# google/dynibar

Measured on NVIDIA H100. Metric: rays/sec (64+64 samples x 8 src views), higher is better.
Workload: dtype bf16

## Files before the change

dynibar_b200/csrc/chains_wg.cu:

```cuda
#include "nets.cuh"
#include "wg_engine.cuh"

namespace dyn {

using namespace tc;
using namespace fe;
using namespace wg;

namespace {

constexpr float kLog2e = 1.4426950408889634f, kLn2 = 0.6931471805599453f;

template <int RING>
struct ChainBars {
  static constexpr int kTileFull = 2 * RING, kTileEmpty = 2 * RING + 1, kCount = 2 * RING + 2;
};

template <int kTile, int kExtra, int kConst, int RING = kWgRing>
struct ChainSmem {
  static constexpr int kTileOff = RING * kWgStage;
  static constexpr int kExtraOff = kTileOff + kTile;
  static constexpr int kConstOff = kExtraOff + kExtra;
  static constexpr int kBarOff = (kConstOff + kConst * 4 + 7) & ~7;
  static constexpr int kBytes = kBarOff + ChainBars<RING>::kCount * 8;
  static_assert(kBytes + kWgMaxChunks * 16 <= 227 * 1024, "shared memory of one CTA");
};

template <int RING = kWgRing>
__device__ __forceinline__ uint32_t chain_init(uint8_t* smem, int bar_off, FusedChunk* s_tab,
                                               const FusedChunk* chunks, int nchunks) {
  const uint32_t bar0 = smem_u32(smem + bar_off);
  stage_chunks(s_tab, chunks, nchunks);
  if (threadIdx.x == 0) {
    for (int i = 0; i < RING; ++i) {
      mbar_init(bar0 + 8u * i, 1);
      mbar_init(bar0 + 8u * (RING + i), 8);
    }
    mbar_init(bar0 + 8u * ChainBars<RING>::kTileFull, 1);
    mbar_init(bar0 + 8u * ChainBars<RING>::kTileEmpty, 8);
    mbar_fence_init();
  }
  return bar0;
}

template <int RING = kWgRing>
__device__ __forceinline__ void chain_producers(const FusedChunk* s_tab, int nchunks, const void* wimg,
                                                const void* src, uint32_t tile_bytes, int n_iter, uint8_t* smem,
                                                uint32_t bar0) {
  setmaxnreg_dec<kProducerRegs>();
  const int t = threadIdx.x & 127;
  if (t == 0) {
    producer_loop<RING, kWgStage>(s_tab, nchunks, wimg, n_iter, smem, bar0);
  } else if (t == 32) {
    const uint8_t* s = reinterpret_cast<const uint8_t*>(src);
    const uint32_t dst = smem_u32(smem + RING * kWgStage);
    uint32_t k = 0;
    for (int it = blockIdx.x; it < n_iter; it += gridDim.x, ++k) {
      if (k > 0) mbar_wait(bar0 + 8u * ChainBars<RING>::kTileEmpty, (k - 1) & 1);
      mbar_arrive_expect_tx(bar0 + 8u * ChainBars<RING>::kTileFull, tile_bytes);
      bulk_g2s(dst, s + (size_t)it * tile_bytes, tile_bytes, bar0 + 8u * ChainBars<RING>::kTileFull);
    }
  }
}
template <int RING = kWgRing>
__device__ __forceinline__ void tile_wait(uint32_t bar0, uint32_t k) {
  mbar_wait(bar0 + 8u * ChainBars<RING>::kTileFull, k & 1);
}
template <int RING = kWgRing>
__device__ __forceinline__ void tile_release(uint32_t bar0) {
  __syncwarp();
  if ((threadIdx.x & 31) == 0) mbar_arrive(bar0 + 8u * ChainBars<RING>::kTileEmpty);
}

__device__ __forceinline__ void bias_afrag(uint32_t* a, int c0, int q) {
  const uint32_t one = q == 0 ? 0x3F803F80u : 0u;
  a[0] = a[1] = c0 == 0 ? one : 0u;
  a[2] = a[3] = c0 == 0 ? 0u : one;
}
template <int NA>
__device__ __forceinline__ void elu_log2_all(float* acc) {
#pragma unroll
  for (int i = 0; i < NA; ++i) acc[i] = elu_log2(acc[i]);
}

__device__ __forceinline__ float2* f32_pair(const void* base, long long row, int c) {
  return reinterpret_cast<float2*>(const_cast<uint8_t*>(reinterpret_cast<const uint8_t*>(base)) +
                                   tile_f32_off(row, c >> 2) + (c & 3) * 4);
}

__device__ __forceinline__ void store_image128(const float* acc, void* img, long long row0, const int* fr, int q,
                                               long long P) {
  uint8_t* o = reinterpret_cast<uint8_t*>(img);
#pragma unroll
  for (int h = 0; h < 2; ++h) {
    const long long row = row0 + fr[h];
    const bool ok = row < P;
#pragma unroll
    for (int j = 0; j < 16; ++j)
      *reinterpret_cast<uint32_t*>(o + tile_image_off(row, j, 16) + 4 * q) =
          ok ? pack_bf16x2(acc[4 * j + 2 * h], acc[4 * j + 2 * h + 1]) : 0u;
  }
}

__device__ __forceinline__ float rows8_max(float v) {
  v = fmaxf(v, __shfl_xor_sync(0xffffffffu, v, 4));
  v = fmaxf(v, __shfl_xor_sync(0xffffffffu, v, 8));
  return fmaxf(v, __shfl_xor_sync(0xffffffffu, v, 16));
}

constexpr int kP1Tile = 34 * 2048;
using P1Smem = ChainSmem<kP1Tile, 0, 0>;

__global__ void __launch_bounds__(kWgThreads, 1) point1_wg_kernel(const __grid_constant__ Point1Args a) {
  extern __shared__ __align__(1024) uint8_t smem[];
  __shared__ __align__(16) FusedChunk s_tab[kWgMaxChunks];
  const uint32_t bar0 = chain_init(smem, P1Smem::kBarOff, s_tab, a.chunks, a.nchunks);
  __syncthreads();
  const int n_iter = (int)((a.P + 127) / 128);
  const int tid = threadIdx.x, lane = tid & 31;
  const int wg = __shfl_sync(0xffffffffu, tid >> 7, 0);
  if (wg == 2) {
    chain_producers(s_tab, a.nchunks, a.wimg, a.G, (uint32_t)kP1Tile, n_iter, smem, bar0);
    return;
  }
  setmaxnreg_inc<kConsumerRegs>();
  const int q = lane & 3, ww = (tid & 127) >> 5;
  const int fr[2] = {16 * ww + (lane >> 2), 16 * ww + (lane >> 2) + 8};
  Ring rg{smem, bar0, 0u, false, 0};
  const uint32_t tile = smem_u32(smem + P1Smem::kTileOff) + 1024u * wg;
  uint32_t k = 0;
  for (int it = blockIdx.x; it < n_iter; it += gridDim.x, ++k) {
    const long long row0 = (long long)it * 128 + 64 * wg;
    float acc[128];
    tile_wait(bar0, k);
    layer_ss<256, 17, 128>(acc, tile, rg);
    layer_finish<256>(acc, rg);
    tile_release(bar0);
    {
      uint32_t af[17][4];
      elu_log2_all<128>(acc);
#pragma unroll
      for (int s = 0; s < 16; ++s) acc_to_afrag(acc, s, af[s]);
      bias_afrag(af[16], 8, q);
      layer_rs<128, 17>(acc, af, rg);
    }
#pragma unroll
    for (int h = 0; h < 2; ++h) {
      const long long row = row0 + fr[h];
      const bool ok = row < a.P;
      const float* pe = a.posenc ? a.posenc + (ok ? row % a.S : 0) * 128 : nullptr;
#pragma unroll
      for (int j = 0; j < 16; ++j) {
        const int c = 8 * j + 2 * q;
        float v0 = elu_from_log2(acc[4 * j + 2 * h]), v1 = elu_from_log2(acc[4 * j + 2 * h + 1]);
        if (pe) {
          const float2 p = __ldg(reinterpret_cast<const float2*>(pe + c));
          v0 += p.x;
          v1 += p.y;
        }
        acc[4 * j + 2 * h] = v0;
        acc[4 * j + 2 * h + 1] = v1;
        if (ok) *f32_pair(a.g2, row, c) = make_float2(v0, v1);
      }
    }
    uint32_t ag[8][4];
    to_afrag<8>(acc, ag);
    layer_rs<128, 8>(acc, ag, rg);
    store_image128(acc, a.Q, row0, fr, q, a.P);
    layer_rs<128, 8>(acc, ag, rg);
    store_image128(acc, a.K, row0, fr, q, a.P);
    layer_rs<128, 8>(acc, ag, rg);
    store_image128(acc, a.V, row0, fr, q, a.P);
  }
}

constexpr int kP2Tile = 16 * 2048;
constexpr int kPePtsBytes = 6 * 1024, kPeDirBytes = 4 * 1024;
constexpr int C_LNW = 0, C_LNB = 128, C_WOG2 = 256, C_WRGB4 = 384, C_BOG2 = 576, C_BRGB4 = 577;
constexpr int kP2Const = 580;
using P2Smem = ChainSmem<kP2Tile, 2 * (kPePtsBytes + kPeDirBytes), kP2Const>;

__device__ __forceinline__ void point2_constants(const Point2Args& a, float* cst, bool dynamic) {
  const int tid = threadIdx.x;
  const float* p = a.params;
  for (int i = tid; i < 128; i += blockDim.x) {
    cst[C_LNW + i] = p[a.o_lnw + i];
    cst[C_LNB + i] = p[a.o_lnb + i];
    cst[C_WOG2 + i] = p[a.o_woutgeo2 + i] * kLn2;
  }
  if (dynamic) {
    for (int i = tid; i < 192; i += blockDim.x) cst[C_WRGB4 + i] = p[a.o_wrgb4 + i] * kLn2;
    if (tid < 3) cst[C_BRGB4 + tid] = p[a.o_brgb4 + tid];
  }
  if (tid == 0) cst[C_BOG2] = p[a.o_boutgeo2];
}

__device__ __forceinline__ void write_pe_tiles(const Point2Args& a, long long row0, uint8_t* pe_pts, uint8_t* pe_dir) {
  const int tw = (threadIdx.x & 127) >> 6, r = threadIdx.x & 63;
  const long long row = row0 + r;
  const bool valid = row < a.P;
  if (tw == 0) {
    float p3[3] = {0.f, 0.f, 0.f};
    if (valid) { p3[0] = a.pts[row * 3]; p3[1] = a.pts[row * 3 + 1]; p3[2] = a.pts[row * 3 + 2]; }
    float pe[48];
    pe_pow2<3, 5>(p3, pe);
    pe[33] = 1.f; pe[34] = 1.f;
#pragma unroll
    for (int i = 35; i < 48; ++i) pe[i] = 0.f;
    uint8_t* arow = pe_pts + (r >> 3) * 128 + (r & 7) * 16;
#pragma unroll
    for (int g = 0; g < 6; ++g) store8_64(arow, 8 * g, pe + 8 * g);
  } else {
    const long long ray = valid ? row / a.S : 0;
    float d3[3] = {a.ray_dir[ray * 3], a.ray_dir[ray * 3 + 1], a.ray_dir[ray * 3 + 2]};
    float pe2[32];
    pe_pow2<3, 4>(d3, pe2);
    pe2[27] = 1.f; pe2[28] = 1.f;
#pragma unroll
    for (int i = 29; i < 32; ++i) pe2[i] = 0.f;
    uint8_t* arow = pe_dir + (r >> 3) * 128 + (r & 7) * 16;
#pragma unroll
    for (int g = 0; g < 4; ++g) store8_64(arow, 8 * g, pe2 + 8 * g);
  }
  fence_proxy_async_smem();
}

template <bool DYNAMIC, class RG>
__device__ __forceinline__ void point2_heads(float* acc, const Point2Args& a, const float* cst, uint32_t pe_pts,
                                             uint32_t pe_dir, const long long* rows, const bool* ok, const float* nv,
                                             int wg, RG& rg) {
  const int q = threadIdx.x & 3;
// ... 740 lines not shown
```

dynibar_b200/csrc/view_wg.cu:

```cuda
#include "geometry.cuh"
#include "nets.cuh"
#include "wg_engine.cuh"

namespace dyn {

using namespace tc;
using namespace fe;
using namespace wg;

namespace {

constexpr int kPeBytes = 14 * 1024, kPoolBytes = 30 * 1024, kWgATile = kPeBytes + kPoolBytes;
constexpr int C_B1 = 0, C_B2 = 256, C_B3 = 304, C_B4 = 560, C_B5 = 688, C_B6 = 816, C_W6V = 944, C_B7 = 1072,
              C_W8 = 1200, C_MISC = 1328, C_DFEAT = 1332, C_CAMS = 1372, C_W1 = 1628, C_MK = 1756, C_TGT = 1884;
constexpr int kWgConst = C_TGT + 3 * kMaxTargets;
constexpr int kViewBars = 2 * kWgRing + 4;
constexpr int kWgSmem = kWgRing * kWgStage + 2 * kWgATile + kWgConst * 4 + 4  + kViewBars * 8;
static_assert(kWgSmem + kWgMaxChunks * 16 <= 227 * 1024, "shared memory of one CTA");
constexpr int kViewThreads = 4 * 128;
constexpr int kViewConsumerRegs = 208, kViewFrontRegs = 72, kViewProducerRegs = 24;

enum Phase {
  PH_FRONT, PH_BAR, PH_WEIGHTS, PH_F1, PH_F1_EPI, PH_F2, PH_F2_EPI, PH_F3, PH_F3_EPI, PH_F4, PH_F4_EPI, PH_F5,
  PH_F5_EPI, PH_F6, PH_F6_EPI, PH_F7, PH_F7_EPI, PH_POOL2, PH_HANDOFF,
  PH_T = 28, PH_W = 29, PH_ITERS = 30, PH_LIFE = 31
};
constexpr int kPhaseSlots = 32;
__shared__ long long s_phase[3][kPhaseSlots];
struct PhaseClock {
  const ViewFusedArgs& a;
  int wg;
  __device__ __forceinline__ bool on() const { return a.dbg != nullptr && blockIdx.x == 0 && (threadIdx.x & 127) == 0; }
  __device__ __forceinline__ long long* c() const { return s_phase[wg]; }
  __device__ __forceinline__ void start() {
    if (!on()) return;
    for (int i = 0; i < kPhaseSlots; ++i) c()[i] = 0;
    c()[PH_T] = c()[PH_LIFE] = clock64();
  }
  __device__ __forceinline__ void mark(int ph, long long waits) {
    if (!on()) return;
    long long* s = c();
    const long long now = clock64();
    s[ph] += now - s[PH_T] - (waits - s[PH_W]);
    s[PH_WEIGHTS] += waits - s[PH_W];
    s[PH_T] = now;
    s[PH_W] = waits;
  }
  __device__ __forceinline__ void iteration() {
    if (on()) ++c()[PH_ITERS];
  }
  __device__ __forceinline__ void finish() {
    if (!on()) return;
    c()[PH_LIFE] = clock64() - c()[PH_LIFE];
    for (int i = 0; i < kPhaseSlots; ++i) a.dbg[kPhaseSlots * wg + i] = c()[i];
  }
};

__device__ __forceinline__ void pe_comp(float x, float* o) {
  float s, c;
  __sincosf(x, &s, &c);
  o[0] = x;
#pragma unroll
  for (int k = 0; k < 5; ++k) {
    o[1 + k] = c;
    o[6 + k] = s;
    const float s2 = 2.f * s * c, c2 = 1.f - 2.f * s * s;
    s = s2; c = c2;
  }
}

template <int KS>
__device__ __forceinline__ void layer_ss256(float* acc, uint32_t a_tile, Ring& rg) {
  layer_issue<256, KS>(acc, rg, [&](float* d, int ks, uint64_t bd, uint32_t sc) {
    const uint64_t ad = smem_desc(a_tile + ks * 2048u, 1024u, 128u);
    Wgmma<128, 0, 0>::mma(d, ad, bd, sc);
    Wgmma<128, 0, 0>::mma(d + 64, ad, bd + (2048u >> 4), sc);
  });
}

template <int N, int KS>
__device__ __forceinline__ void layer_rs_issue(float* acc, const uint32_t (&af)[KS][4], Ring& rg) {
  layer_issue<N, KS>(acc, rg, [&](float* d, int ks, uint64_t bd, uint32_t sc) { WgmmaRS<N>::mma(d, af[ks], bd, sc); });
}

__device__ __forceinline__ void named_bar_arrive(int id, int nthreads) {
  asm volatile("bar.arrive %0, %1;" ::"r"(id), "r"(nthreads) : "memory");
}

__device__ __forceinline__ void store2_64(uint8_t* tile, int r, int col, float x, float y) {
  *reinterpret_cast<uint32_t*>(tile + (col >> 3) * 1024 + (r >> 3) * 128 + (r & 7) * 16 + (col & 7) * 2) =
      pack_bf16x2(x, y);
}

template <int VP, bool ST, bool MC>
__device__ __forceinline__ void front_end(const ViewFusedArgs& a, const float* cst, int t, long long row0,
                                          uint8_t* pe_tile, uint8_t* pool_tile, float* s_w1, float* s_mk) {
  const int tw = t >> 6, r = t & 63, v = r & (VP - 1);
  uint8_t* arow_pe = pe_tile + (r >> 3) * 128 + (r & 7) * 16;
  uint8_t* arow_pool = pool_tile + (r >> 3) * 128 + (r & 7) * 16;
  const float wh = a.w_img, hh = a.h_img;
  const bool want_rgb = (tw == 0) || (ST && a.mask_rgb);

  const long long pl = (row0 + r) / VP;
  const bool pt_ok = pl < a.P;
  const bool valid = pt_ok && v < a.V;
  const long long m = pl * a.V + v;
  float p3[3] = {0.f, 0.f, 0.f};
  if (pt_ok) { p3[0] = a.pts[pl * 3]; p3[1] = a.pts[pl * 3 + 1]; p3[2] = a.pts[pl * 3 + 2]; }
  float q3[3] = {p3[0], p3[1], p3[2]};
  if (!ST && valid) {
    const float* qq = a.pts_seq + ((long long)v * a.seq_stride + pl) * 3;
    q3[0] = qq[0]; q3[1] = qq[1]; q3[2] = qq[2];
  }

  const int vc = valid ? v : 0;
  const float* cam = cst + C_CAMS + 16 * vc;
  float pu, pv;
  bool front;
  project_point(cam, q3[0], q3[1], q3[2], pu, pv, front);
  const bool inb = (pu <= wh - 1.f) && (pu >= 0.f) && (pv <= hh - 1.f) && (pv >= 0.f);
  const float mask_proj = (valid && inb && front) ? 1.f : 0.f;

  float chv[24];
#pragma unroll
  for (int i = 0; i < 24; ++i) chv[i] = 0.f;
  float rgb[3] = {0.f, 0.f, 0.f};
  {
    const float gx = 2.f * pu / (wh - 1.f) - 1.f, gy = 2.f * pv / (hh - 1.f) - 1.f;
    const float fx = (gx + 1.f) * 0.5f * (float)(a.w - 1), fy = (gy + 1.f) * 0.5f * (float)(a.h - 1);
    const float x0f = floorf(fx), y0f = floorf(fy);
    const int x0 = (int)x0f, y0 = (int)y0f;
    const float ax = fx - x0f, ay = fy - y0f, bx = (x0f + 1.f) - fx, by = (y0f + 1.f) - fy;
    const uint16_t* base = a.feat_bf + (long long)vc * a.h * a.w * kC + 16 * tw;
#pragma unroll
    for (int dy = 0; dy < 2; ++dy) {
      uint4 tf[4];
      float tw4[2];
#pragma unroll
      for (int dx = 0; dx < 2; ++dx) {
        const int xi = x0 + dx, yi = y0 + dy;
        const bool in = valid && xi >= 0 && xi < a.w && yi >= 0 && yi < a.h;
        tw4[dx] = in ? (dx ? ax : bx) * (dy ? ay : by) : 0.f;
        const int xc = min(max(xi, 0), a.w - 1), yc = min(max(yi, 0), a.h - 1);
        const uint4* tp = reinterpret_cast<const uint4*>(base + ((long long)yc * a.w + xc) * kC);
        tf[2 * dx] = __ldg(tp);
        tf[2 * dx + 1] = __ldg(tp + 1);
      }
#pragma unroll
      for (int dx = 0; dx < 2; ++dx) {
#pragma unroll
        for (int hlf = 0; hlf < 2; ++hlf) {
          const uint4 qv = tf[2 * dx + hlf];
          const uint32_t u[4] = {qv.x, qv.y, qv.z, qv.w};
#pragma unroll
          for (int j = 0; j < 4; ++j) {
            const float lo = __uint_as_float(u[j] << 16), hi = __uint_as_float(u[j] & 0xffff0000u);
            if (tw == 0) {
              chv[3 + 8 * hlf + 2 * j] += lo * tw4[dx];
              chv[3 + 8 * hlf + 2 * j + 1] += hi * tw4[dx];
            } else {
              chv[8 * hlf + 2 * j] += lo * tw4[dx]; chv[8 * hlf + 2 * j + 1] += hi * tw4[dx];
            }
          }
        }
      }
    }
    if (want_rgb) {
      const float fx = (gx + 1.f) * 0.5f * (float)(a.W - 1), fy = (gy + 1.f) * 0.5f * (float)(a.H - 1);
      const float x0f = floorf(fx), y0f = floorf(fy);
      const int x0 = (int)x0f, y0 = (int)y0f;
      const float ax = fx - x0f, ay = fy - y0f, bx = (x0f + 1.f) - fx, by = (y0f + 1.f) - fy;
      const float* base = a.rgba + (long long)vc * a.H * a.W * 4;
      float4 tr[4];
      float twr[4];
#pragma unroll
      for (int dy = 0; dy < 2; ++dy)
#pragma unroll
        for (int dx = 0; dx < 2; ++dx) {
          const int xi = x0 + dx, yi = y0 + dy;
          const bool in = valid && xi >= 0 && xi < a.W && yi >= 0 && yi < a.H;
          twr[2 * dy + dx] = in ? (dx ? ax : bx) * (dy ? ay : by) : 0.f;
          const int xc = min(max(xi, 0), a.W - 1), yc = min(max(yi, 0), a.H - 1);
          tr[2 * dy + dx] = __ldg(reinterpret_cast<const float4*>(base + ((long long)yc * a.W + xc) * 4));
        }
#pragma unroll
      for (int tp = 0; tp < 4; ++tp) {
        rgb[0] += tr[tp].x * twr[tp]; rgb[1] += tr[tp].y * twr[tp]; rgb[2] += tr[tp].z * twr[tp];
      }
    }
  }

  float rd[4];
  {
    const float* tgt = a.cams.tgt;
    if (MC) tgt = cst + C_TGT + 3 * (pt_ok ? a.tgt_idx[(int)pl / a.S] : 0);
    float a0 = tgt[0] - p3[0], a1 = tgt[1] - p3[1], a2 = tgt[2] - p3[2];
    normalize3(a0, a1, a2);
    float b0 = cam[12] - q3[0], b1 = cam[13] - q3[1], b2 = cam[14] - q3[2];
    normalize3(b0, b1, b2);
    rd[0] = a0 - b0; rd[1] = a1 - b1; rd[2] = a2 - b2;
    rd[3] = a0 * b0 + a1 * b1 + a2 * b2;
    normalize3(rd[0], rd[1], rd[2]);
  }

  float mask = mask_proj;
  if (ST && a.mask_rgb) mask *= ((rgb[0] + rgb[1] + rgb[2]) > 1e-3f) ? 1.f : 0.f;
  if (tw == 0) {
    chv[0] = rgb[0]; chv[1] = rgb[1]; chv[2] = rgb[2];
    if (valid) {
      a.mask_proj[m] = mask_proj;
      if (ST) {
        a.mask_eff[m] = mask;
        reinterpret_cast<float4*>(a.ray_diff)[m] = make_float4(rd[0], rd[1], rd[2], rd[3]);
        a.rgb_in[m * 3] = rgb[0]; a.rgb_in[m * 3 + 1] = rgb[1]; a.rgb_in[m * 3 + 2] = rgb[2];
      }
    }
  }
  if (!ST) {
    const int c0 = tw == 0 ? 0 : 19, nc = tw == 0 ? 19 : 16;
#pragma unroll
    for (int i = 0; i < 19; ++i)
      if (i < nc) chv[i] = valid ? chv[i] + cst[C_DFEAT + c0 + i] : 0.f;
  }

  float w1;
  if (ST && a.anti_alias) {
    const float e = ex2f(cst[C_MISC + 2] * (rd[3] - 1.f) * 1.4426950408889634f);
    const float emin = group_min<VP>(valid ? e : INFINITY);
    w1 = valid ? (e - emin) * mask : 0.f;
  } else {
    w1 = mask;
  }
  w1 = w1 / (group_sum<VP>(w1) + 1e-8f);
  if (tw == 0) { s_w1[r] = w1; s_mk[r] = mask; }

#pragma unroll
  for (int g = 0; g < 3; ++g) {
    if (tw == 1 && g == 2) break;
    float o[24];
#pragma unroll
    for (int j = 0; j < 8; ++j) {
      const float fv = chv[8 * g + j];
      const float s1 = group_sum<VP>(w1 * fv);
      const float d = fv - s1;
      const float s2 = group_sum<VP>(w1 * d * d);
      o[j] = s1; o[8 + j] = s2; o[16 + j] = fv;
    }
    const int cb = 72 * tw + 24 * g;
    store8_64(arow_pool, cb, o);
    store8_64(arow_pool, cb + 8, o + 8);
    store8_64(arow_pool, cb + 16, o + 16);
  }
  if (!ST && tw == 1) {
    const float z[8] = {0.f, 0.f, 0.f, 0.f, 0.f, 0.f, 0.f, 0.f};
    store8_64(arow_pool, 120, z);
  }

  if (ST) {
    float pl6[6];
    {
      const float ox = cam[12], oy = cam[13], oz = cam[14];
      float dx = p3[0] - ox, dy = p3[1] - oy, dz = p3[2] - oz;
      normalize3(dx, dy, dz);
      pl6[0] = dx; pl6[1] = dy; pl6[2] = dz;
      pl6[3] = oy * dz - oz * dy;
      pl6[4] = oz * dx - ox * dz;
      pl6[5] = ox * dy - oy * dx;
    }
    float xin[56];
    if (tw == 0) {
      pe_comp(p3[0], xin);         store8_64(arow_pe, 0, xin);
      pe_comp(p3[1], xin + 11);    store8_64(arow_pe, 8, xin + 8);
      pe_comp(p3[2], xin + 22);    store8_64(arow_pe, 16, xin + 16); store8_64(arow_pe, 24, xin + 24);
      pe_comp(pl6[0], xin + 33);   store8_64(arow_pe, 32, xin + 32);
      pe_comp(pl6[1], xin + 44);   xin[55] = 0.f;
      store8_64(arow_pe, 40, xin + 40);  store8_64(arow_pe, 48, xin + 48);
    } else {
      pe_comp(pl6[2], xin);        store8_64(arow_pe, 56, xin);
      pe_comp(pl6[3], xin + 11);   store8_64(arow_pe, 64, xin + 8);
      pe_comp(pl6[4], xin + 22);   store8_64(arow_pe, 72, xin + 16); store8_64(arow_pe, 80, xin + 24);
      pe_comp(pl6[5], xin + 33);   store8_64(arow_pe, 88, xin + 32);
      xin[44] = rd[0]; xin[45] = rd[1]; xin[46] = rd[2]; xin[47] = rd[3];
#pragma unroll
      for (int i = 48; i < 56; ++i) xin[i] = 0.f;
      store8_64(arow_pe, 96, xin + 40);  store8_64(arow_pe, 104, xin + 48);
    }
  }
}

template <int VP, bool ST, bool MC>
__global__ void __launch_bounds__(kViewThreads, 1) view_wg_kernel(const __grid_constant__ ViewFusedArgs a) {
  static_assert(ST || !MC, "multi-camera launches are static-net only");
  extern __shared__ __align__(1024) uint8_t smem[];
  uint8_t* ring = smem;
  uint8_t* atiles = smem + kWgRing * kWgStage;
  float* cst = reinterpret_cast<float*>(atiles + 2 * kWgATile);
  uint64_t* bars = reinterpret_cast<uint64_t*>(smem + ((kWgRing * kWgStage + 2 * kWgATile + kWgConst * 4 + 7) & ~7));
  __shared__ __align__(16) FusedChunk s_tab[kWgMaxChunks];
  const int tid = threadIdx.x, lane = tid & 31;
  const int wg = __shfl_sync(0xffffffffu, tid >> 7, 0);
  const uint32_t bar0 = smem_u32(bars);
  const uint32_t tiles_full = bar0 + 8u * (2 * kWgRing), tiles_empty = tiles_full + 16u;
  stage_chunks(s_tab, a.chunks, a.nchunks);
  if (tid == 0) {
    for (int i = 0; i < kWgRing; ++i) {
      mbar_init(bar0 + 8u * i, 1);
      mbar_init(bar0 + 8u * (kWgRing + i), 8);
    }
    for (int c = 0; c < 2; ++c) {
      mbar_init(tiles_full + 8u * c, 128);
      mbar_init(tiles_empty + 8u * c, 4);
    }
    mbar_fence_init();
  }
  {
    const float* prm = a.params;
    for (int i = tid; i < 256; i += blockDim.x) {
      const int vv = i >> 4, j = i & 15;
      cst[C_CAMS + i] = j < 12 ? a.cams.P[vv][j] : (j < 15 ? a.cams.center[vv][j - 12] : 0.f);
      cst[C_B1 + i] = ST ? prm[a.o_b1 + i] : 0.f;
      cst[C_B3 + i] = prm[a.o_b3 + i];
    }
    for (int i = tid; i < 128; i += blockDim.x) {
      cst[C_B4 + i] = prm[a.o_b4 + i];
      cst[C_B5 + i] = prm[a.o_b5 + i];
      cst[C_B6 + i] = prm[a.o_b6 + i];
      cst[C_W6V + i] = prm[a.o_w6 + 128 * 128 + i];
      cst[C_B7 + i] = prm[a.o_b7 + i];
      cst[C_W8 + i] = prm[a.o_w8 + i];
    }
    if (tid < 48) cst[C_B2 + tid] = (ST && tid < kF) ? prm[a.o_b2 + tid] : 0.f;
    if (tid < 40) cst[C_DFEAT + tid] = (!ST && tid < kF) ? a.dfeat[tid] : 0.f;
    if (tid == 0) {
      cst[C_MISC + 0] = prm[a.o_b6 + 128];
      cst[C_MISC + 1] = prm[a.o_b8];
      cst[C_MISC + 2] = (ST && a.o_s >= 0) ? fabsf(prm[a.o_s]) : 0.f;
    }
    if (MC && tid < 3 * kMaxTargets) cst[C_TGT + tid] = a.cams.tgts[tid / 3][tid % 3];
  }
  __syncthreads();

  const long long n_rows = a.P * VP;
  const int n_iter = (int)((n_rows + 127) / 128);
  const int t = tid & 127;
  if (wg == 3) {
    setmaxnreg_dec<kViewProducerRegs>();
    if (t == 0) producer_loop<kWgRing, kWgStage>(s_tab, a.nchunks, a.wimg, n_iter, ring, bar0);
    return;
  }
  if (wg == 2) {
    setmaxnreg_dec<kViewFrontRegs>();
    PhaseClock pc{a, 2};
    pc.start();
    uint32_t k = 0;
    for (int it = blockIdx.x; it < n_iter; it += gridDim.x, ++k) {
#pragma unroll 1
      for (int c = 0; c < 2; ++c) {
        if (k > 0) mbar_wait(tiles_empty + 8u * c, (k - 1) & 1);
        pc.mark(PH_HANDOFF, 0);
        front_end<VP, ST, MC>(a, cst, t, (long long)it * 128 + 64 * c, atiles + c * kWgATile,
                          atiles + c * kWgATile + kPeBytes, cst + C_W1 + 64 * c, cst + C_MK + 64 * c);
        fence_proxy_async_smem();
        mbar_arrive(tiles_full + 8u * c);
        pc.mark(PH_FRONT, 0);
      }
      pc.iteration();
    }
    pc.finish();
    return;
  }
  setmaxnreg_inc<kViewConsumerRegs>();

  const int ww = t >> 5, q = lane & 3;
  uint8_t* pool_tile = atiles + wg * kWgATile + kPeBytes;
  const uint32_t pe_addr = smem_u32(atiles + wg * kWgATile), pool_addr = smem_u32(pool_tile);
  const float* s_w1 = cst + C_W1 + 64 * wg;
  const float* s_mk = cst + C_MK + 64 * wg;
  const int fr[2] = {16 * ww + (lane >> 2), 16 * ww + (lane >> 2) + 8};

  PhaseClock pc{a, wg};
  Ring rg{ring, bar0, 0u, pc.on(), 0};
  pc.start();
#define TS(ph) pc.mark(ph, rg.wait_cycles)
  auto in_turn = [&](auto issue, bool pass) {
    named_bar_sync(3 + wg, 256);
    TS(PH_BAR);
    issue();
    if (pass) named_bar_arrive(4 - wg, 256);
  };
  if (wg == 1) named_bar_arrive(3, 256);

  uint32_t k = 0;
  for (int it = blockIdx.x; it < n_iter; it += gridDim.x, ++k) {
    const long long row0 = (long long)it * 128 + 64 * wg;
    mbar_wait(tiles_full + 8u * wg, k & 1);
    TS(PH_HANDOFF);
    const float w1r[2] = {s_w1[fr[0]], s_w1[fr[1]]}, mk[2] = {s_mk[fr[0]], s_mk[fr[1]]};

    float acc[128];
    if (ST) {
      in_turn([&] { layer_ss256<7>(acc, pe_addr, rg); }, true);
      layer_finish<256>(acc, rg);
      TS(PH_F1);
      {
        uint32_t af[16][4];
        bias_elu<256>(acc, cst + C_B1, q);
        to_afrag<16>(acc, af);
        TS(PH_F1_EPI);
        in_turn([&] { layer_rs_issue<48, 16>(acc, af, rg); }, true);
        layer_finish<48>(acc, rg);
      }
      TS(PH_F2);
      float f[2][10];
#pragma unroll
      for (int h = 0; h < 2; ++h) {
        const long long prow = (row0 + fr[h]) / VP;
        const bool ok = prow < a.P && ((fr[h] & (VP - 1)) < a.V);
        const float* rf = a.ref_feat + (ok ? prow / a.S : 0) * kF;
#pragma unroll
        for (int j = 0; j < 5; ++j)
#pragma unroll
          for (int e = 0; e < 2; ++e) {
            const int n = 8 * j + 2 * q + e;
            f[h][2 * j + e] = (ok && n < kF) ? (acc[4 * j + 2 * h + e] + cst[C_B2 + n]) * __ldg(rf + n) : 0.f;
          }
      }
#pragma unroll
      for (int j = 0; j < 5; ++j) {
        float mu[2][2], va[2][2];
#pragma unroll
        for (int e = 0; e < 2; ++e) {
          const int i = 2 * j + e;
          float tv[2] = {w1r[0] * f[0][i], w1r[1] * f[1][i]}, s1[2], s2[2];
          views_sum<VP>(tv, s1);
          const float d0 = f[0][i] - s1[0], d1 = f[1][i] - s1[1];
          tv[0] = w1r[0] * d0 * d0;
          tv[1] = w1r[1] * d1 * d1;
          views_sum<VP>(tv, s2);
          mu[0][e] = s1[0]; mu[1][e] = s1[1]; va[0][e] = s2[0]; va[1][e] = s2[1];
        }
        const int n = 8 * j + 2 * q;
#pragma unroll
        for (int h = 0; h < 2; ++h) {
          store2_64(pool_tile, fr[h], 120 + n, mu[h][0], mu[h][1]);
          store2_64(pool_tile, fr[h], 160 + n, va[h][0], va[h][1]);
          store2_64(pool_tile, fr[h], 200 + n, f[h][2 * j], f[h][2 * j + 1]);
        }
      }
      TS(PH_F2_EPI);
      fence_proxy_async_smem();
      named_bar_sync(1 + wg, 128);
      TS(PH_BAR);
    }
    in_turn([&] { layer_ss256<ST ? 15 : 8>(acc, pool_addr, rg); }, true);
    layer_finish<256>(acc, rg);
    __syncwarp();
    if (lane == 0) mbar_arrive(tiles_empty + 8u * wg);
    TS(PH_F3);
    {
      uint32_t af[16][4];
      bias_elu<256>(acc, cst + C_B3, q);
      to_afrag<16>(acc, af);
      TS(PH_F3_EPI);
      in_turn([&] { layer_rs_issue<128, 16>(acc, af, rg); }, true);
      layer_finish<128>(acc, rg);
    }
    TS(PH_F4);
    float x[64];
    bias_elu<128>(acc, cst + C_B4, q);
#pragma unroll
    for (int i = 0; i < 64; ++i) x[i] = acc[i];
    {
      uint32_t af[8][4];
      to_afrag<8>(x, af);
      TS(PH_F4_EPI);
      in_turn([&] { layer_rs_issue<128, 8>(acc, af, rg); }, true);
      layer_finish<128>(acc, rg);
    }
    TS(PH_F5);
    float part[2] = {0.f, 0.f};
#pragma unroll
    for (int j = 0; j < 16; ++j) {
      const float2 b = *reinterpret_cast<const float2*>(cst + C_B5 + 8 * j + 2 * q);
      const float2 wv = *reinterpret_cast<const float2*>(cst + C_W6V + 8 * j + 2 * q);
#pragma unroll
      for (int h = 0; h < 2; ++h) {
        float& h0 = acc[4 * j + 2 * h];
        float& h1 = acc[4 * j + 2 * h + 1];
        h0 = elu_fast(fmaf(h0, w1r[h], b.x));
        h1 = elu_fast(fmaf(h1, w1r[h], b.y));
        part[h] = fmaf(h1, wv.y, fmaf(h0, wv.x, part[h]));
      }
    }
    part[0] = quad_sum(part[0]);
    part[1] = quad_sum(part[1]);
    {
      uint32_t af[8][4];
      to_afrag<8>(acc, af);
      TS(PH_F5_EPI);
      in_turn([&] { layer_rs_issue<128, 8>(acc, af, rg); }, true);
      layer_finish<128>(acc, rg);
    }
    TS(PH_F6);
    float vis1[2];
#pragma unroll
    for (int h = 0; h < 2; ++h) vis1[h] = sigmoid_fast(elu_fast(cst[C_MISC + 0] + part[h])) * mk[h];
    bias_elu<128>(acc, cst + C_B6, q);
#pragma unroll
    for (int i = 0; i < 64; ++i) x[i] += acc[i];
    {
      uint32_t af[8][4];
      to_afrag<8>(x, af);
      if (ST) {
        uint8_t* xo = reinterpret_cast<uint8_t*>(a.X);
#pragma unroll
        for (int s = 0; s < 8; ++s)
#pragma unroll
          for (int k = 0; k < 4; ++k)
            *reinterpret_cast<uint32_t*>(xo + tile_image_off(row0 + fr[k & 1], 2 * s + (k >> 1), 16) + 4 * q) = af[s][k];
      }
      TS(PH_F6_EPI);
      in_turn([&] { layer_rs_issue<128, 8>(acc, af, rg); }, wg == 0 || it + (int)gridDim.x < n_iter);
      layer_finish<128>(acc, rg);
    }
    TS(PH_F7);
    float p7[2] = {0.f, 0.f};
#pragma unroll
    for (int j = 0; j < 16; ++j) {
      const float2 b = *reinterpret_cast<const float2*>(cst + C_B7 + 8 * j + 2 * q);
      const float2 wv = *reinterpret_cast<const float2*>(cst + C_W8 + 8 * j + 2 * q);
#pragma unroll
      for (int h = 0; h < 2; ++h) {
        p7[h] = fmaf(elu_fast(fmaf(acc[4 * j + 2 * h], vis1[h], b.x)), wv.x, p7[h]);
        p7[h] = fmaf(elu_fast(fmaf(acc[4 * j + 2 * h + 1], vis1[h], b.y)), wv.y, p7[h]);
      }
    }
    float vis2[2];
#pragma unroll
    for (int h = 0; h < 2; ++h) {
      vis2[h] = sigmoid_fast(cst[C_MISC + 1] + quad_sum(p7[h])) * mk[h];
      const long long prow = (row0 + fr[h]) / VP;
      const int vh = fr[h] & (VP - 1);
      if (ST && q == 0 && prow < a.P && vh < a.V) a.vis2[prow * a.V + vh] = vis2[h];
    }
    TS(PH_F7_EPI);

    float vsum[2], w2[2], Wsum[2], nval[2];
    views_sum<VP>(vis2, vsum);
#pragma unroll
    for (int h = 0; h < 2; ++h) w2[h] = vis2[h] / (vsum[h] + 1e-8f);
    views_sum<VP>(w2, Wsum);
    views_sum<VP>(mk, nval);
    const bool b4 = lane & 16, b3 = lane & 8, b2 = lane & 4;
    const int j0 = (b4 ? 8 : 0) + (b3 ? 4 : 0) + (b2 ? 2 : 0);
    uint8_t* gi = reinterpret_cast<uint8_t*>(a.G);
#pragma unroll
    for (int pi = 0; pi < (VP == 8 ? 2 : 1); ++pi) {
      float st4[2][4];
#pragma unroll
      for (int qq = 0; qq < 2; ++qq) {
        float s32[32], s16[16], s8[8];
#pragma unroll
        for (int j = 0; j < 16; ++j)
#pragma unroll
          for (int e = 0; e < 2; ++e) {
            const float x0 = x[4 * j + e], x1 = x[4 * j + 2 + e];
            if (VP == 16)
              s32[2 * j + e] = qq ? w2[0] * x0 * x0 + w2[1] * x1 * x1 : w2[0] * x0 + w2[1] * x1;
            else
              s32[2 * j + e] = pi ? (qq ? w2[1] * x1 * x1 : w2[1] * x1) : (qq ? w2[0] * x0 * x0 : w2[0] * x0);
          }
        rs_step<32>(s32, s16, b4, 16);
        rs_step<16>(s16, s8, b3, 8);
        rs_step<8>(s8, st4[qq], b2, 4);
      }
      const long long prow = (row0 + 16 * ww + 8 * pi) / VP;
      if (prow < a.P) {
        const float W = Wsum[pi];
        float mu4[4], vr4[4];
#pragma unroll
        for (int i = 0; i < 4; ++i) {
          mu4[i] = st4[0][i];
          vr4[i] = st4[1][i] - mu4[i] * mu4[i] * (2.f - W);
        }
#pragma unroll
        for (int k = 0; k < 2; ++k) {
          const int c = 8 * (j0 + k) + 2 * q;
          *reinterpret_cast<uint32_t*>(gi + tile_image_off(prow, c >> 3, 34) + (c & 7) * 2) =
              pack_bf16x2(mu4[2 * k], mu4[2 * k + 1]);
          *reinterpret_cast<uint32_t*>(gi + tile_image_off(prow, 16 + (c >> 3), 34) + (c & 7) * 2) =
              pack_bf16x2(vr4[2 * k], vr4[2 * k + 1]);
        }
        if (lane == 0) {
          *reinterpret_cast<uint4*>(gi + tile_image_off(prow, 32, 34)) = make_uint4(pack_bf16x2(W / (float)a.V, 0.f), 0u, 0u, 0u);
          *reinterpret_cast<uint4*>(gi + tile_image_off(prow, 33, 34)) = make_uint4(0x3F803F80u, 0u, 0u, 0u);
          a.nvalid[prow] = nval[pi];
        }
      }
    }
    TS(PH_POOL2);
    pc.iteration();
  }
#undef TS
  pc.finish();
}

}

size_t view_wg_bytes(int kind) { (void)kind; return (size_t)(512 * 1024); }

int view_wg_build(dyn_net* n, const float* P, void* dst_dev, size_t dst_bytes, cudaStream_t st) {
  std::vector<uint8_t> img;
  std::vector<FusedChunk> tab;
  auto add = [&](const LinearP& l, int N, int Npad, int Kpad, std::vector<int> map) {
    HostLayer L;
    L.W = P + l.w; L.N = N; L.Kw = l.in; L.Npad = Npad; L.Kpad = Kpad; L.colmap = std::move(map);
    append_wg_layer(L, img, tab);
  };
  auto gathered_map = [](std::vector<int>& m, int C) {
    for (int s = 0; s < 19; ++s) {
      const int b = 24 * (s / 8) + (s % 8);
      m[b] = s; m[b + 8] = C + s; m[b + 16] = 2 * C + s;
    }
    for (int s = 0; s < 16; ++s) {
      const int c = 19 + s, b = 72 + 24 * (s / 8) + (s % 8);
      m[b] = c; m[b + 8] = C + c; m[b + 16] = 2 * C + c;
    }
  };
  if (n->kind == DYN_NET_STATIC) {
    const StaticLayout& L = n->sl;
    std::vector<int> m1(112, -1);
    auto comp_col = [](int ci, int j) {
      if (ci < 3) return j == 0 ? ci : (j <= 5 ? 3 + 3 * (j - 1) + ci : 18 + 3 * (j - 6) + ci);
      const int d = ci - 3;
      return j == 0 ? 33 + d : (j <= 5 ? 39 + 6 * (j - 1) + d : 69 + 6 * (j - 6) + d);
    };
    for (int ci = 0; ci < 5; ++ci)
      for (int j = 0; j < 11; ++j) m1[11 * ci + j] = comp_col(ci, j);
    for (int ci = 5; ci < 9; ++ci)
      for (int j = 0; j < 11; ++j) m1[56 + 11 * (ci - 5) + j] = comp_col(ci, j);
    for (int i = 0; i < 4; ++i) m1[100 + i] = 99 + i;
    add(L.ray_dir0, 256, 256, 112, m1);
    add(L.ray_dir2, kF, 48, 256, identity_map(256, 256));
    std::vector<int> m3(240, -1);
    gathered_map(m3, 70);
    for (int c = 0; c < kF; ++c) {
      m3[120 + c] = 35 + c; m3[160 + c] = 70 + 35 + c; m3[200 + c] = 140 + 35 + c;
    }
    add(L.base0, 256, 256, 240, m3);
  } else {
    const DynamicLayout& L = n->dl;
    std::vector<int> m3(128, -1);
    gathered_map(m3, kF);
    add(L.base0, 256, 256, 128, m3);
  }
  const LinearP& base2 = n->kind == DYN_NET_STATIC ? n->sl.base2 : n->dl.base2;
  const LinearP& vis0 = n->kind == DYN_NET_STATIC ? n->sl.vis0 : n->dl.vis0;
  const LinearP& vis2 = n->kind == DYN_NET_STATIC ? n->sl.vis2 : n->dl.vis2;
  const LinearP& vis2_0 = n->kind == DYN_NET_STATIC ? n->sl.vis2_0 : n->dl.vis2_0;
  add(base2, 128, 128, 256, identity_map(256, 256));
  add(vis0, 128, 128, 128, identity_map(128, 128));
  add(vis2, 128, 128, 128, identity_map(128, 128));
  add(vis2_0, 128, 128, 128, identity_map(128, 128));
  return upload_wg_image(img, tab, dst_dev, dst_bytes, "per-view", &n->wg, st);
}

int launch_view_wg(const dyn_net* n, ViewFusedArgs& a, int V, cudaStream_t st) {
  if (n->wg.img == nullptr) return fail(DYN_E_INVALID, "net has no per-view weight images");
  a.wimg = n->wg.img;
  a.chunks = n->wg.tab;
  a.nchunks = n->wg.nchunks;
  static int sms = 0;
  if (sms == 0) {
    int dev = 0;
    DYN_CUDA(cudaGetDevice(&dev));
    DYN_CUDA(cudaDeviceGetAttribute(&sms, cudaDevAttrMultiProcessorCount, dev));
#define PREP_WG(VPV, STV, MCV) \
    DYN_CUDA(cudaFuncSetAttribute(view_wg_kernel<VPV, STV, MCV>, cudaFuncAttributeMaxDynamicSharedMemorySize, kWgSmem))
    PREP_WG(8, true, false); PREP_WG(16, true, false); PREP_WG(8, false, false); PREP_WG(16, false, false);
    PREP_WG(8, true, true); PREP_WG(16, true, true);
#undef PREP_WG
  }
  const bool st_net = n->kind == DYN_NET_STATIC;
  const bool mc = a.tgt_idx != nullptr;
  if (mc && !st_net) return fail(DYN_E_INVALID, "multi-camera per-view launches are for the static net only");
  const int VP = V <= 8 ? 8 : 16;
  const long long n_iter = (a.P * VP + 127) / 128;
  const int grid = (int)(n_iter < sms ? n_iter : sms);
  if (grid == 0) return DYN_OK;
  ProfScope prof(st_net ? PROF_VIEW_ST : PROF_VIEW_DY, st);
  if (st_net && mc) {
    if (VP == 8) view_wg_kernel<8, true, true><<<grid, kViewThreads, kWgSmem, st>>>(a);
    else view_wg_kernel<16, true, true><<<grid, kViewThreads, kWgSmem, st>>>(a);
  } else if (st_net) {
    if (VP == 8) view_wg_kernel<8, true, false><<<grid, kViewThreads, kWgSmem, st>>>(a);
    else view_wg_kernel<16, true, false><<<grid, kViewThreads, kWgSmem, st>>>(a);
  } else {
    if (VP == 8) view_wg_kernel<8, false, false><<<grid, kViewThreads, kWgSmem, st>>>(a);
    else view_wg_kernel<16, false, false><<<grid, kViewThreads, kWgSmem, st>>>(a);
  }
  DYN_LAUNCH_CHECK();
  return DYN_OK;
}

}
```

dynibar_b200/csrc/wg_engine.cuh:

```cuda
#pragma once
#include <vector>

#include "fused_engine.cuh"

namespace dyn {
namespace wg {

using namespace tc;
using namespace fe;

constexpr int kWgRing = 8;
constexpr int kWgStage = 16384;
constexpr int kWgThreads = 3 * 128;
constexpr int kConsumerRegs = 232, kProducerRegs = 40;
constexpr int kWgMaxChunks = 72;

__host__ __device__ constexpr int wg_chunk_ksteps(int N) { return kWgStage / (N * 32) < 8 ? kWgStage / (N * 32) : 8; }

__device__ __forceinline__ void store8_64(uint8_t* arow, int c0, const float* v) {
  *reinterpret_cast<uint4*>(arow + (c0 >> 3) * 1024) =
      make_uint4(pack_bf16x2(v[0], v[1]), pack_bf16x2(v[2], v[3]), pack_bf16x2(v[4], v[5]), pack_bf16x2(v[6], v[7]));
}

template <int RING>
struct RingN {
  uint8_t* base;
  uint32_t bar0;
  uint32_t cnt;
  bool prof;
  long long wait_cycles;
  __device__ __forceinline__ uint32_t wait_full(uint32_t c) {
    const uint32_t st = c % RING;
    const long long t0 = prof ? clock64() : 0;
    mbar_wait(bar0 + 8u * st, (c / RING) & 1);
    if (prof) wait_cycles += clock64() - t0;
    return smem_u32(base + st * kWgStage);
  }
  __device__ __forceinline__ void release(uint32_t c) {
    __syncwarp();
    if ((threadIdx.x & 31) == 0) mbar_arrive(bar0 + 8u * (RING + c % RING));
  }
};
using Ring = RingN<kWgRing>;

template <int N, int KS, class RG, class Mma>
__device__ __forceinline__ void layer_issue(float* acc, RG& rg, Mma mma) {
  constexpr int KC = wg_chunk_ksteps(N), NCH = (KS + KC - 1) / KC;
  fence_regs<N / 2>(acc);
  wgmma_fence();
#pragma unroll
  for (int c = 0; c < NCH; ++c) {
    const uint32_t w = rg.wait_full(rg.cnt + c);
#pragma unroll
    for (int s = 0; s < KC; ++s)
      if (c * KC + s < KS) mma(acc, c * KC + s, smem_desc(w + s * N * 32u, N * 16u, 128u), (c | s) ? 1u : 0u);
    wgmma_commit();
    if (c > 0) {
      wgmma_wait<1>();
      rg.release(rg.cnt + c - 1);
    }
  }
  rg.cnt += NCH;
}
template <int N, class RG>
__device__ __forceinline__ void layer_finish(float* acc, RG& rg) {
  wgmma_wait<0>();
  fence_regs<N / 2>(acc);
  rg.release(rg.cnt - 1);
}

template <int N, int KS, int ROWS = 64, class RG>
__device__ __forceinline__ void layer_ss(float* acc, uint32_t a_tile, RG& rg) {
  layer_issue<N, KS>(acc, rg, [&](float* d, int ks, uint64_t bd, uint32_t sc) {
    Wgmma<N, 0, 0>::mma(d, smem_desc(a_tile + ks * (ROWS * 32u), ROWS * 16u, 128u), bd, sc);
  });
}
template <int N, int KS, class RG>
__device__ __forceinline__ void layer_rs(float* acc, const uint32_t (&af)[KS][4], RG& rg) {
  layer_issue<N, KS>(acc, rg, [&](float* d, int ks, uint64_t bd, uint32_t sc) { WgmmaRS<N>::mma(d, af[ks], bd, sc); });
  layer_finish<N>(acc, rg);
}
template <int N, int KS, int KR, class RG>
__device__ __forceinline__ void layer_rs_ss(float* acc, const uint32_t (*af)[4], uint32_t tile64, RG& rg) {
  layer_issue<N, KS>(acc, rg, [&](float* d, int ks, uint64_t bd, uint32_t sc) {
    if (ks < KR) WgmmaRS<N>::mma(d, af[ks < KR ? ks : 0], bd, sc);
    else Wgmma<N, 0, 0>::mma(d, smem_desc(tile64 + (ks - KR) * 2048u, 1024u, 128u), bd, sc);
  });
  layer_finish<N>(acc, rg);
}

template <int N>
__device__ __forceinline__ void bias_relu(float* acc, const float* bias, int q) {
#pragma unroll
  for (int j = 0; j < N / 8; ++j) {
    const float2 b = *reinterpret_cast<const float2*>(bias + 8 * j + 2 * q);
#pragma unroll
    for (int h = 0; h < 2; ++h) {
      acc[4 * j + 2 * h] = fmaxf(acc[4 * j + 2 * h] + b.x, 0.f);
      acc[4 * j + 2 * h + 1] = fmaxf(acc[4 * j + 2 * h + 1] + b.y, 0.f);
    }
  }
}
template <int N>
__device__ __forceinline__ void bias_elu(float* acc, const float* bias, int q) {
#pragma unroll
  for (int j = 0; j < N / 8; ++j) {
    const float2 b = *reinterpret_cast<const float2*>(bias + 8 * j + 2 * q);
#pragma unroll
    for (int h = 0; h < 2; ++h) {
      acc[4 * j + 2 * h] = elu_fast(acc[4 * j + 2 * h] + b.x);
      acc[4 * j + 2 * h + 1] = elu_fast(acc[4 * j + 2 * h + 1] + b.y);
    }
  }
}
template <int KS>
__device__ __forceinline__ void to_afrag(const float* acc, uint32_t (&af)[KS][4]) {
#pragma unroll
  for (int s = 0; s < KS; ++s) acc_to_afrag(acc, s, af[s]);
}
__device__ __forceinline__ float quad_sum(float v) {
  v += __shfl_xor_sync(0xffffffffu, v, 1);
  return v + __shfl_xor_sync(0xffffffffu, v, 2);
}
__device__ __forceinline__ float rows8_sum(float v) {
  v += __shfl_xor_sync(0xffffffffu, v, 4);
  v += __shfl_xor_sync(0xffffffffu, v, 8);
  return v + __shfl_xor_sync(0xffffffffu, v, 16);
}
template <int VP>
__device__ __forceinline__ void views_sum(const float* v, float* s) {
  if (VP == 16) {
    s[0] = s[1] = rows8_sum(v[0] + v[1]);
  } else {
    s[0] = rows8_sum(v[0]);
    s[1] = rows8_sum(v[1]);
  }
}

inline void append_wg_layer(const HostLayer& L, std::vector<uint8_t>& img, std::vector<FusedChunk>& tab) {
  append_block(L, img, tab, 0, 0, 0, 0, kWgStage, 0, L.Kpad / 16);
}

inline int upload_wg_image(const std::vector<uint8_t>& img, const std::vector<FusedChunk>& tab, void* dst_dev,
                           size_t dst_bytes, const char* what, ChainImage* out, cudaStream_t st) {
  const size_t img_bytes = (img.size() + 255) & ~(size_t)255;
  const size_t need = img_bytes + tab.size() * sizeof(FusedChunk);
  if (need > dst_bytes) return fail(DYN_E_INVALID, "%s images need %zu bytes, have %zu", what, need, dst_bytes);
  if (tab.size() > (size_t)kWgMaxChunks) return fail(DYN_E_INVALID, "%s chunk table too long (%zu)", what, tab.size());
  DYN_CUDA(cudaMemcpyAsync(dst_dev, img.data(), img.size(), cudaMemcpyHostToDevice, st));
  DYN_CUDA(cudaMemcpyAsync(reinterpret_cast<char*>(dst_dev) + img_bytes, tab.data(), tab.size() * sizeof(FusedChunk),
                           cudaMemcpyHostToDevice, st));
  DYN_CUDA(cudaStreamSynchronize(st));
  out->img = dst_dev;
  out->tab = reinterpret_cast<const FusedChunk*>(reinterpret_cast<char*>(dst_dev) + img_bytes);
  out->nchunks = (int)tab.size();
  return DYN_OK;
}

}
}
```

Before: 239,300.

## Fold layer biases into WGMMA via constant-one K columns and pipeline first-layer epilogue

```diff
diff --git a/dynibar_b200/csrc/chains_wg.cu b/dynibar_b200/csrc/chains_wg.cu
--- a/dynibar_b200/csrc/chains_wg.cu
+++ b/dynibar_b200/csrc/chains_wg.cu
@@ -72,11 +72,6 @@
   if ((threadIdx.x & 31) == 0) mbar_arrive(bar0 + 8u * ChainBars<RING>::kTileEmpty);
 }
 
-__device__ __forceinline__ void bias_afrag(uint32_t* a, int c0, int q) {
-  const uint32_t one = q == 0 ? 0x3F803F80u : 0u;
-  a[0] = a[1] = c0 == 0 ? one : 0u;
-  a[2] = a[3] = c0 == 0 ? 0u : one;
-}
 template <int NA>
 __device__ __forceinline__ void elu_log2_all(float* acc) {
 #pragma unroll
diff --git a/dynibar_b200/csrc/view_wg.cu b/dynibar_b200/csrc/view_wg.cu
--- a/dynibar_b200/csrc/view_wg.cu
+++ b/dynibar_b200/csrc/view_wg.cu
@@ -11,8 +11,8 @@
 namespace {
 
 constexpr int kPeBytes = 14 * 1024, kPoolBytes = 30 * 1024, kWgATile = kPeBytes + kPoolBytes;
-constexpr int C_B1 = 0, C_B2 = 256, C_B3 = 304, C_B4 = 560, C_B5 = 688, C_B6 = 816, C_W6V = 944, C_B7 = 1072,
-              C_W8 = 1200, C_MISC = 1328, C_DFEAT = 1332, C_CAMS = 1372, C_W1 = 1628, C_MK = 1756, C_TGT = 1884;
+constexpr int C_B5 = 0, C_W6V = 128, C_B7 = 256, C_W8 = 384, C_MISC = 512, C_DFEAT = 516, C_CAMS = 556, C_W1 = 812,
+              C_MK = 940, C_TGT = 1068;
 constexpr int kWgConst = C_TGT + 3 * kMaxTargets;
 constexpr int kViewBars = 2 * kWgRing + 4;
 constexpr int kWgSmem = kWgRing * kWgStage + 2 * kWgATile + kWgConst * 4 + 4  + kViewBars * 8;
@@ -252,7 +252,7 @@
     store8_64(arow_pool, cb + 16, o + 16);
   }
   if (!ST && tw == 1) {
-    const float z[8] = {0.f, 0.f, 0.f, 0.f, 0.f, 0.f, 0.f, 0.f};
+    const float z[8] = {1.f, 1.f, 0.f, 0.f, 0.f, 0.f, 0.f, 0.f};
     store8_64(arow_pool, 120, z);
   }
 
@@ -281,8 +281,9 @@
       pe_comp(pl6[4], xin + 22);   store8_64(arow_pe, 72, xin + 16); store8_64(arow_pe, 80, xin + 24);
       pe_comp(pl6[5], xin + 33);   store8_64(arow_pe, 88, xin + 32);
       xin[44] = rd[0]; xin[45] = rd[1]; xin[46] = rd[2]; xin[47] = rd[3];
-#pragma unroll
-      for (int i = 48; i < 56; ++i) xin[i] = 0.f;
+      xin[48] = 1.f; xin[49] = 1.f;
+#pragma unroll
+      for (int i = 50; i < 56; ++i) xin[i] = 0.f;
       store8_64(arow_pe, 96, xin + 40);  store8_64(arow_pe, 104, xin + 48);
     }
   }
@@ -318,18 +319,13 @@
     for (int i = tid; i < 256; i += blockDim.x) {
       const int vv = i >> 4, j = i & 15;
       cst[C_CAMS + i] = j < 12 ? a.cams.P[vv][j] : (j < 15 ? a.cams.center[vv][j - 12] : 0.f);
-      cst[C_B1 + i] = ST ? prm[a.o_b1 + i] : 0.f;
-      cst[C_B3 + i] = prm[a.o_b3 + i];
     }
     for (int i = tid; i < 128; i += blockDim.x) {
-      cst[C_B4 + i] = prm[a.o_b4 + i];
       cst[C_B5 + i] = prm[a.o_b5 + i];
-      cst[C_B6 + i] = prm[a.o_b6 + i];
       cst[C_W6V + i] = prm[a.o_w6 + 128 * 128 + i];
       cst[C_B7 + i] = prm[a.o_b7 + i];
       cst[C_W8 + i] = prm[a.o_w8 + i];
     }
-    if (tid < 48) cst[C_B2 + tid] = (ST && tid < kF) ? prm[a.o_b2 + tid] : 0.f;
     if (tid < 40) cst[C_DFEAT + tid] = (!ST && tid < kF) ? a.dfeat[tid] : 0.f;
     if (tid == 0) {
       cst[C_MISC + 0] = prm[a.o_b6 + 128];
@@ -382,12 +378,17 @@
   Ring rg{ring, bar0, 0u, pc.on(), 0};
   pc.start();
 #define TS(ph) pc.mark(ph, rg.wait_cycles)
+  constexpr bool kRsTurns = !ST;
   auto in_turn = [&](auto issue, bool pass) {
     named_bar_sync(3 + wg, 256);
     TS(PH_BAR);
     issue();
     if (pass) named_bar_arrive(4 - wg, 256);
   };
+  auto rs_turn = [&](auto issue, bool pass) {
+    if (kRsTurns) in_turn(issue, pass);
+    else issue();
+  };
   if (wg == 1) named_bar_arrive(3, 256);
 
   uint32_t k = 0;
@@ -399,18 +400,6 @@
 
     float acc[128];
     if (ST) {
-      in_turn([&] { layer_ss256<7>(acc, pe_addr, rg); }, true);
-      layer_finish<256>(acc, rg);
-      TS(PH_F1);
-      {
-        uint32_t af[16][4];
-        bias_elu<256>(acc, cst + C_B1, q);
-        to_afrag<16>(acc, af);
-        TS(PH_F1_EPI);
-        in_turn([&] { layer_rs_issue<48, 16>(acc, af, rg); }, true);
-        layer_finish<48>(acc, rg);
-      }
-      TS(PH_F2);
       float f[2][10];
 #pragma unroll
       for (int h = 0; h < 2; ++h) {
@@ -422,9 +411,33 @@
 #pragma unroll
           for (int e = 0; e < 2; ++e) {
             const int n = 8 * j + 2 * q + e;
-            f[h][2 * j + e] = (ok && n < kF) ? (acc[4 * j + 2 * h + e] + cst[C_B2 + n]) * __ldg(rf + n) : 0.f;
+            f[h][2 * j + e] = (ok && n < kF) ? __ldg(rf + n) : 0.f;
           }
       }
+      in_turn([&] { layer_ss256<7>(acc, pe_addr, rg); }, true);
+      layer_finish<256>(acc, rg);
+      TS(PH_F1);
+      float acc2[24];
+      {
+        uint32_t af[17][4];
+        layer_issue<48, 17>(acc2, rg, [&](float* d, int ks, uint64_t bd, uint32_t sc) {
+          if (ks < 16) {
+            elu_all<16>(acc + 8 * ks);
+            acc_to_afrag(acc, ks, af[ks]);
+          } else {
+            bias_afrag(af[16], 0, q);
+          }
+          wgmma_fence();
+          WgmmaRS<48>::mma(d, af[ks], bd, sc);
+        });
+        TS(PH_F1_EPI);
+        layer_finish<48>(acc2, rg);
+      }
+      TS(PH_F2);
+#pragma unroll
+      for (int h = 0; h < 2; ++h)
+#pragma unroll
+        for (int i = 0; i < 10; ++i) f[h][i] *= acc2[4 * (i >> 1) + 2 * h + (i & 1)];
 #pragma unroll
       for (int j = 0; j < 5; ++j) {
         float mu[2][2], va[2][2];
@@ -440,11 +453,12 @@
           mu[0][e] = s1[0]; mu[1][e] = s1[1]; va[0][e] = s2[0]; va[1][e] = s2[1];
         }
         const int n = 8 * j + 2 * q;
+        const bool ones = j == 4 && q == 3;
 #pragma unroll
         for (int h = 0; h < 2; ++h) {
           store2_64(pool_tile, fr[h], 120 + n, mu[h][0], mu[h][1]);
           store2_64(pool_tile, fr[h], 160 + n, va[h][0], va[h][1]);
-          store2_64(pool_tile, fr[h], 200 + n, f[h][2 * j], f[h][2 * j + 1]);
+          store2_64(pool_tile, fr[h], 200 + n, ones ? 1.f : f[h][2 * j], ones ? 1.f : f[h][2 * j + 1]);
         }
       }
       TS(PH_F2_EPI);
@@ -452,29 +466,31 @@
       named_bar_sync(1 + wg, 128);
       TS(PH_BAR);
     }
-    in_turn([&] { layer_ss256<ST ? 15 : 8>(acc, pool_addr, rg); }, true);
+    in_turn([&] { layer_ss256<ST ? 15 : 8>(acc, pool_addr, rg); }, kRsTurns || wg == 0 || it + (int)gridDim.x < n_iter);
     layer_finish<256>(acc, rg);
     __syncwarp();
     if (lane == 0) mbar_arrive(tiles_empty + 8u * wg);
     TS(PH_F3);
     {
-      uint32_t af[16][4];
-      bias_elu<256>(acc, cst + C_B3, q);
-      to_afrag<16>(acc, af);
+      uint32_t af[17][4];
+      elu_all<256>(acc);
+#pragma unroll
+      for (int s = 0; s < 16; ++s) acc_to_afrag(acc, s, af[s]);
+      bias_afrag(af[16], 0, q);
       TS(PH_F3_EPI);
-      in_turn([&] { layer_rs_issue<128, 16>(acc, af, rg); }, true);
+      rs_turn([&] { layer_rs_issue<128, 17>(acc, af, rg); }, true);
       layer_finish<128>(acc, rg);
     }
     TS(PH_F4);
     float x[64];
-    bias_elu<128>(acc, cst + C_B4, q);
+    elu_all<128>(acc);
 #pragma unroll
     for (int i = 0; i < 64; ++i) x[i] = acc[i];
     {
       uint32_t af[8][4];
       to_afrag<8>(x, af);
       TS(PH_F4_EPI);
-      in_turn([&] { layer_rs_issue<128, 8>(acc, af, rg); }, true);
+      rs_turn([&] { layer_rs_issue<128, 8>(acc, af, rg); }, true);
       layer_finish<128>(acc, rg);
     }
     TS(PH_F5);
@@ -495,17 +511,19 @@
     part[0] = quad_sum(part[0]);
     part[1] = quad_sum(part[1]);
     {
-      uint32_t af[8][4];
-      to_afrag<8>(acc, af);
+      uint32_t af[9][4];
+#pragma unroll
+      for (int s = 0; s < 8; ++s) acc_to_afrag(acc, s, af[s]);
+      bias_afrag(af[8], 0, q);
       TS(PH_F5_EPI);
-      in_turn([&] { layer_rs_issue<128, 8>(acc, af, rg); }, true);
+      rs_turn([&] { layer_rs_issue<128, 9>(acc, af, rg); }, true);
       layer_finish<128>(acc, rg);
     }
     TS(PH_F6);
     float vis1[2];
 #pragma unroll
     for (int h = 0; h < 2; ++h) vis1[h] = sigmoid_fast(elu_fast(cst[C_MISC + 0] + part[h])) * mk[h];
-    bias_elu<128>(acc, cst + C_B6, q);
+    elu_all<128>(acc);
 #pragma unroll
     for (int i = 0; i < 64; ++i) x[i] += acc[i];
     {
@@ -520,7 +538,7 @@
             *reinterpret_cast<uint32_t*>(xo + tile_image_off(row0 + fr[k & 1], 2 * s + (k >> 1), 16) + 4 * q) = af[s][k];
       }
       TS(PH_F6_EPI);
-      in_turn([&] { layer_rs_issue<128, 8>(acc, af, rg); }, wg == 0 || it + (int)gridDim.x < n_iter);
+      rs_turn([&] { layer_rs_issue<128, 8>(acc, af, rg); }, wg == 0 || it + (int)gridDim.x < n_iter);
       layer_finish<128>(acc, rg);
     }
     TS(PH_F7);
@@ -612,10 +630,16 @@
 int view_wg_build(dyn_net* n, const float* P, void* dst_dev, size_t dst_bytes, cudaStream_t st) {
   std::vector<uint8_t> img;
   std::vector<FusedChunk> tab;
-  auto add = [&](const LinearP& l, int N, int Npad, int Kpad, std::vector<int> map) {
+  auto add = [&](const LinearP& l, int N, int Npad, int Kpad, std::vector<int> map, bool fold_bias) {
     HostLayer L;
     L.W = P + l.w; L.N = N; L.Kw = l.in; L.Npad = Npad; L.Kpad = Kpad; L.colmap = std::move(map);
+    if (fold_bias) L.bias = P + l.b;
     append_wg_layer(L, img, tab);
+  };
+  auto bias_kstep = [](int K) {
+    std::vector<int> m = identity_map(K, K + 16);
+    m[K] = kBiasHi; m[K + 1] = kBiasLo;
+    return m;
   };
   auto gathered_map = [](std::vector<int>& m, int C) {
     for (int s = 0; s < 19; ++s) {
@@ -640,28 +664,31 @@
     for (int ci = 5; ci < 9; ++ci)
       for (int j = 0; j < 11; ++j) m1[56 + 11 * (ci - 5) + j] = comp_col(ci, j);
     for (int i = 0; i < 4; ++i) m1[100 + i] = 99 + i;
-    add(L.ray_dir0, 256, 256, 112, m1);
-    add(L.ray_dir2, kF, 48, 256, identity_map(256, 256));
+    m1[104] = kBiasHi; m1[105] = kBiasLo;
+    add(L.ray_dir0, 256, 256, 112, m1, true);
+    add(L.ray_dir2, kF, 48, 272, bias_kstep(256), true);
     std::vector<int> m3(240, -1);
     gathered_map(m3, 70);
     for (int c = 0; c < kF; ++c) {
       m3[120 + c] = 35 + c; m3[160 + c] = 70 + 35 + c; m3[200 + c] = 140 + 35 + c;
     }
-    add(L.base0, 256, 256, 240, m3);
+    m3[238] = kBiasHi; m3[239] = kBiasLo;
+    add(L.base0, 256, 256, 240, m3, true);
   } else {
     const DynamicLayout& L = n->dl;
     std::vector<int> m3(128, -1);
     gathered_map(m3, kF);
-    add(L.base0, 256, 256, 128, m3);
+    m3[120] = kBiasHi; m3[121] = kBiasLo;
+    add(L.base0, 256, 256, 128, m3, true);
   }
   const LinearP& base2 = n->kind == DYN_NET_STATIC ? n->sl.base2 : n->dl.base2;
   const LinearP& vis0 = n->kind == DYN_NET_STATIC ? n->sl.vis0 : n->dl.vis0;
   const LinearP& vis2 = n->kind == DYN_NET_STATIC ? n->sl.vis2 : n->dl.vis2;
   const LinearP& vis2_0 = n->kind == DYN_NET_STATIC ? n->sl.vis2_0 : n->dl.vis2_0;
-  add(base2, 128, 128, 256, identity_map(256, 256));
-  add(vis0, 128, 128, 128, identity_map(128, 128));
-  add(vis2, 128, 128, 128, identity_map(128, 128));
-  add(vis2_0, 128, 128, 128, identity_map(128, 128));
+  add(base2, 128, 128, 272, bias_kstep(256), true);
+  add(vis0, 128, 128, 128, identity_map(128, 128), false);
+  add(vis2, 128, 128, 144, bias_kstep(128), true);
+  add(vis2_0, 128, 128, 128, identity_map(128, 128), false);
   return upload_wg_image(img, tab, dst_dev, dst_bytes, "per-view", &n->wg, st);
 }
 
diff --git a/dynibar_b200/csrc/wg_engine.cuh b/dynibar_b200/csrc/wg_engine.cuh
--- a/dynibar_b200/csrc/wg_engine.cuh
+++ b/dynibar_b200/csrc/wg_engine.cuh
@@ -102,16 +102,14 @@
   }
 }
 template <int N>
-__device__ __forceinline__ void bias_elu(float* acc, const float* bias, int q) {
+__device__ __forceinline__ void elu_all(float* acc) {
 #pragma unroll
-  for (int j = 0; j < N / 8; ++j) {
-    const float2 b = *reinterpret_cast<const float2*>(bias + 8 * j + 2 * q);
-#pragma unroll
-    for (int h = 0; h < 2; ++h) {
-      acc[4 * j + 2 * h] = elu_fast(acc[4 * j + 2 * h] + b.x);
-      acc[4 * j + 2 * h + 1] = elu_fast(acc[4 * j + 2 * h + 1] + b.y);
-    }
-  }
+  for (int i = 0; i < N / 2; ++i) acc[i] = elu_fast(acc[i]);
+}
+__device__ __forceinline__ void bias_afrag(uint32_t* a, int c0, int q) {
+  const uint32_t one = q == 0 ? 0x3F803F80u : 0u;
+  a[0] = a[1] = c0 == 0 ? one : 0u;
+  a[2] = a[3] = c0 == 0 ? 0u : one;
 }
 template <int KS>
 __device__ __forceinline__ void to_afrag(const float* acc, uint32_t (&af)[KS][4]) {
```

Measured after the change: 245,300 (median of 6 runs). 1.02x the previous value.
